# zeyadmohamedabdo/Visual-Question-Answering-VQA-system

Hardware: AMD Instinct MI355X
Metric: image-question pairs/sec (train step) (higher is better)
Workload: dtype bf16; 1 GPU; VQA train step fwd+CE+bwd+allreduce+clip+AdamW, batch 512/GPU, 3x224x224 images, 20 tokens, d=256, 4 text layers, 49 image tokens, 1000 answers, dropout on (BASELINE configs[2]); batch_per_gpu=512, global_batch=512, parallelism=dp1, reducer=off

## Files before the change

include/vqa_hip.h:

```cpp
#ifndef VQA_HIP_H
#define VQA_HIP_H
#include <stdint.h>
#ifdef __cplusplus
extern "C" {
#endif
typedef struct ihipStream_t* hipStream_t;

int vqa_igemm_mtiles(int M, int N, int loader);
int vqa_igemm_variant(int dtype, int loader, int M, int N, int Kw, int B, int H, int W, int C, int Ho, int Wo,
                      int R, int S, int stride, int pad);
int vqa_igemm(int dtype, int loader, const void* a, const void* w, void* out, const float* bias, const void* addend,
              const void* addmask, const void* outmask , float* stats, int M, int N, int Kw, int B, int H, int W, int C, int Ho, int Wo,
              int R, int S, int stride, int pad, int transposed, int relu, float drop_p, unsigned long long drop_seed,
              int stats_mode ,
              hipStream_t stream);
int vqa_linear_dgrad_act(int dtype, const void* dz, const void* wt, void* dx, const void* addend, const void* outact, float drop_p,
                         int M, int Kin, int N, hipStream_t stream);
int vqa_wgrad_plan(int dtype, int loader, int M, int N, int Kw, int B, int H, int W, int C, int R, int S, long long* ws_floats,
                   int* kind, int* tile_n, int* tile_k, int* nsplit);
int vqa_wgrad(int dtype, int loader, const void* dy, const void* x, float* dw, int M, int N, int Kw, int B, int H, int W,
              int C, int Ho, int Wo, int R, int S, int stride, int pad, float* ws, long long ws_floats, hipStream_t stream);
int vqa_pack_rows(int dtype, const float* in, void* out, int N, int K, int Kp, hipStream_t stream);
int vqa_pack_transpose(int dtype, const float* in, void* out, int N, int T, int C, int ldo, int col0, int flip, hipStream_t stream);
int vqa_pack_transpose_batch(int dtype, const float* flat, void* out, const long long* desc, int nd, int total_blocks, hipStream_t stream);
int vqa_fold_bn_batch(int dtype, const float* flat, void* wout, float* bout, const long long* desc, int nd, int total_blocks, float eps, hipStream_t stream);
int vqa_mx_quant(int dtype, const void* in, uint8_t* q, uint8_t* s, int M, int C, hipStream_t stream);
int vqa_fold_bn_mxfp8(const float* flat, uint8_t* wq, uint8_t* ws, float* bout, const long long* desc, int nd, int total_blocks, float eps,
                      hipStream_t stream);
int vqa_conv_mxfp8(const uint8_t* a, const uint8_t* as, const uint8_t* w, const uint8_t* ws, const float* bias, const void* addend,
                   void* out, uint8_t* oq, uint8_t* os, int M, int N, int B, int H, int W, int C, int Ho, int Wo, int R, int S,
                   int stride, int pad, int relu, hipStream_t stream);
int vqa_conv3x3_c64p_blocks(int B, int H, int W);
int vqa_conv3x3_c64p_bnred(const void* x, const void* w, void* out, const void* bn_y, const float* bn_coef, unsigned long long* bn_facc,
                           int B, int H, int W, hipStream_t stream);
int vqa_conv3x3_c64p_epi(const void* x, const void* w, void* out, const void* addend, const void* addmask, const void* outmask,
                         int B, int H, int W, hipStream_t stream);
int vqa_conv3x3_c64p(const void* x, const void* w, void* out, float* stats, int B, int H, int W,
                     int stats_mode , hipStream_t stream);
int vqa_gemm8p(const void* A, const void* B, void* C, int M, int N, int K, hipStream_t stream);
int vqa_gemm4w(const void* A, const void* B, void* C, int M, int N, int K, hipStream_t stream);
int vqa_conv8p_ok(int B, int H, int W, int C, int N);
int vqa_conv8p(const void* x, const void* w, void* out, unsigned long long* stats,
               const void* addend, const void* addmask, const void* outmask ,
               const void* bn_y, const float* bn_coef, unsigned long long* bn_facc ,
               int bn_selfmask ,
               const void* bn_y2, const float* bn_coef2 ,
               int B, int H, int W, int C, int N, int transposed, int stride , hipStream_t stream);
int vqa_conv3x3_c64p_bn(const void* y, const unsigned long long* acc, const float* gamma, const float* beta, float* running_mean,
                        float* running_var, long long* num_batches_tracked, float* coef_out, const void* w, void* out, float* stats,
                        int B, int H, int W, int stats_mode, double count, float momentum, float eps, hipStream_t stream);
int vqa_wgrad3x3_c64_bn_ok(int B, int H, int W);
int vqa_wgrad3x3_c64_bn(const void* y, const float* coef, const void* dy, float* dw , int B, int H, int W,
                        float* ws , long long ws_floats, hipStream_t stream);
int vqa_wgrad3x3_c128_blocks(int B, int H, int W);
int vqa_wgrad3x3_c128(const void* x, const void* dy, float* dw, int B, int H, int W, float* ws, long long ws_floats, hipStream_t stream);
int vqa_wgrad3x3_c64_blocks(int B, int H, int W);
int vqa_wgrad3x3_c64(const void* x, const void* dy, float* dw , int B, int H, int W,
                     float* ws ,
                     long long ws_floats, hipStream_t stream);
long long vqa_wgrad_group_ws(int dtype, int njobs, const int* M, const int* N, const int* Kw);
int vqa_wgrad_group(int dtype, int njobs, const void* const* dy, const void* const* x, float* const* dw, const int* M, const int* N,
                    const int* Kw, float* ws, long long ws_floats, hipStream_t stream);
int vqa_slab_reduce(const float* ws, float* dw, int nslabs, long long n, hipStream_t stream);
int vqa_dgrad_s2(int dtype, const void* dy, const void* dyd, const void* wt, void* out, int B, int H, int W, int C,
                 int Ho, int Wo, int N, int R, int pad, hipStream_t stream);
int vqa_stem_conv_blocks(int B, int H, int W);
int vqa_stem_pack(const float* w_krsc, void* wstem, hipStream_t stream);
int vqa_stem_conv(const float* img, const void* wstem, void* out, float* stats, int B, int H, int W, hipStream_t stream);
int vqa_stem_conv_pool_ok(int B, int H, int W);
int vqa_stem_conv_pool(const float* img, const void* wstem, const float* coef, void* out, int B, int H, int W, hipStream_t stream);
int vqa_stem_wgrad_blocks(int B, int H, int W);
int vqa_stem_wgrad(const float* img, const void* dy, float* dw , int B, int H, int W,
                   float* ws , long long ws_floats, hipStream_t stream);
int vqa_stem_wgrad_fused(const float* img, const void* y, const void* dpool, const uint8_t* idx, const float* coef,
                         const float* bcoef, float* dw, int B, int H, int W, float* ws, long long ws_floats, hipStream_t stream);
int vqa_u8_norm_table(float mean0, float mean1, float mean2, float std0, float std1, float std2, void* table, hipStream_t stream);
int vqa_stem_conv_u8(const uint8_t* img_hwc, const void* wstem, void* out, float* stats, int B, int H, int W, const void* table,
                     hipStream_t stream);
int vqa_stem_conv_pool_u8(const uint8_t* img_hwc, const void* wstem, const float* coef, void* out, int B, int H, int W, const void* table,
                          hipStream_t stream);
int vqa_stem_wgrad_u8(const uint8_t* img_hwc, const void* dy, float* dw, int B, int H, int W, float* ws, long long ws_floats,
                      const void* table, hipStream_t stream);
int vqa_stem_wgrad_fused_u8(const uint8_t* img_hwc, const void* y, const void* dpool, const uint8_t* idx, const float* coef,
                            const float* bcoef, float* dw, int B, int H, int W, float* ws, long long ws_floats, const void* table,
                            hipStream_t stream);
int vqa_stem_dgrad_pack(int dtype, const float* w_krsc, void* wpk, hipStream_t stream);
int vqa_stem_dgrad(int dtype, const void* dy, const void* wpk, float* dimg, int B, int H, int W, hipStream_t stream);
int vqa_stem_dgrad_fused_ok(int B, int H, int W);
int vqa_stem_dgrad_fused(const void* y, const void* dpool, const uint8_t* idx, const float* coef, const float* bcoef, const void* wpk,
                         float* dimg, int B, int H, int W, hipStream_t stream);

int vqa_bn_stats_finalize(const float* part, int tiles, int C, double count, const float* gamma, const float* beta,
                          float* running_mean, float* running_var, long long* num_batches_tracked, float momentum, float eps,
                          double* scratch , float* coef, hipStream_t stream);
int vqa_bn_eval_coef(int C, const float* gamma, const float* beta, const float* running_mean, const float* running_var,
                     float eps, float* coef, hipStream_t stream);
int vqa_bn_apply(int dtype, const void* y, const float* coef, const void* res, const float* rcoef, void* out,
                 long long numel, int C, int relu, hipStream_t stream);
int vqa_bn_apply_pool_chunks(int dtype, int HW, int C);
int vqa_bn_apply_pool(int dtype, const void* y, const float* coef, const void* res, const float* rcoef, void* out, int B, int HW, int C,
                      int relu, float* part, hipStream_t stream);
int vqa_bn_acc_words(int K, int C);
int vqa_bn_apply_acc(int dtype, const void* y, const unsigned long long* acc, const float* gamma, const float* beta, float* running_mean,
                     float* running_var, long long* num_batches_tracked, float* coef_out, const void* res,
                     const unsigned long long* racc, const float* rgamma, const float* rbeta, float* rrunning_mean, float* rrunning_var,
                     long long* rnum_batches_tracked, float* rcoef_out, void* out, int B, int HW, int C, int relu, double count,
                     float momentum, float eps, float* pool_part, hipStream_t stream);
int vqa_bn_bwd_blocks(long long rows);
int vqa_bn_bwd_reduce(int dtype, const void* dout, const void* outact, const void* y, const float* coef, const void* y2,
                      const float* coef2, float* slab , long long rows,
                      int C, int self_mask , int acc_mode, hipStream_t stream);
int vqa_bn_bwd_apply_acc(int dtype, const void* dout, const void* outact, const void* y, const unsigned long long* facc, const float* gamma,
                         const float* coef, float* dgamma, float* dbeta, void* dy, const void* y2, const float* gamma2, const float* coef2,
                         float* dgamma2, float* dbeta2, void* dy2, long long numel, int C, double count, int self_mask, hipStream_t stream);
int vqa_bn_bwd_finalize(const float* slab, int nblk, int C, int which, double count, const float* gamma, const float* coef,
                        int training, float* dgamma, float* dbeta, float* bcoef , hipStream_t stream);
int vqa_bn_bwd_apply(int dtype, const void* dout, const void* outact, const void* y, const float* bcoef, void* dy,
                     const void* y2, const float* bcoef2, void* dy2, long long numel, int C, const float* mask_coef ,
// ... 213 lines not shown
```

visual-question-answering-vqa-system_amd/_lib.py:

```python
from __future__ import annotations

import ctypes as C
import os

import torch

_HERE = os.path.dirname(os.path.abspath(__file__))
LIB_PATH = os.path.join(_HERE, "libvqa_hip.so")

P, I, F, D, LL, ULL = C.c_void_p, C.c_int, C.c_float, C.c_double, C.c_longlong, C.c_ulonglong

SIGNATURES = {
    "vqa_gemm8p": [P, P, P, I, I, I, P],
    "vqa_gemm4w": [P, P, P, I, I, I, P],
    "vqa_conv8p_ok": [I, I, I, I, I],
    "vqa_conv8p": [P, P, P, P, P, P, P, P, P, P, I, P, P, I, I, I, I, I, I, I, P],
    "vqa_igemm_mtiles": [I, I, I],
    "vqa_igemm_variant": [I] * 15,
    "vqa_igemm": [I, I, P, P, P, P, P, P, P, P] + [I] * 15 + [F, ULL, I, P],
    "vqa_linear_dgrad_act": [I, P, P, P, P, P, F, I, I, I, P],
    "vqa_wgrad_plan": [I] * 11 + [P, P, P, P, P],
    "vqa_wgrad": [I, I, P, P, P] + [I] * 13 + [P, LL, P],
    "vqa_pack_rows": [I, P, P, I, I, I, P],
    "vqa_pack_transpose": [I, P, P, I, I, I, I, I, I, P],
    "vqa_pack_transpose_batch": [I, P, P, P, I, I, P],
    "vqa_fold_bn_batch": [I, P, P, P, P, I, I, F, P],
    "vqa_mx_quant": [I, P, P, P, I, I, P],
    "vqa_fold_bn_mxfp8": [P, P, P, P, P, I, I, F, P],
    "vqa_conv_mxfp8": [P] * 9 + [I] * 13 + [P],
    "vqa_conv3x3_c64p_blocks": [I, I, I],
    "vqa_conv3x3_c64p": [P, P, P, P, I, I, I, I, P],
    "vqa_conv3x3_c64p_epi": [P, P, P, P, P, P, I, I, I, P],
    "vqa_conv3x3_c64p_bnred": [P, P, P, P, P, P, I, I, I, P],
    "vqa_conv3x3_c64p_bn": [P, P, P, P, P, P, P, P, P, P, P, I, I, I, I, D, F, F, P],
    "vqa_wgrad3x3_c64_bn_ok": [I, I, I],
    "vqa_wgrad3x3_c64_bn": [P, P, P, P, I, I, I, P, LL, P],
    "vqa_wgrad3x3_c128_blocks": [I, I, I],
    "vqa_wgrad3x3_c128": [P, P, P, I, I, I, P, LL, P],
    "vqa_wgrad3x3_c64_blocks": [I, I, I],
    "vqa_wgrad3x3_c64": [P, P, P, I, I, I, P, LL, P],
    "vqa_wgrad_group_ws": [I, I, P, P, P],
    "vqa_wgrad_group": [I, I, P, P, P, P, P, P, P, LL, P],
    "vqa_slab_reduce": [P, P, I, LL, P],
    "vqa_dgrad_s2": [I, P, P, P, P, I, I, I, I, I, I, I, I, I, P],
    "vqa_stem_conv_blocks": [I, I, I],
    "vqa_stem_pack": [P, P, P],
    "vqa_stem_conv": [P, P, P, P, I, I, I, P],
    "vqa_stem_conv_pool_ok": [I, I, I],
    "vqa_stem_conv_pool": [P, P, P, P, I, I, I, P],
    "vqa_stem_wgrad_blocks": [I, I, I],
    "vqa_stem_wgrad": [P, P, P, I, I, I, P, LL, P],
    "vqa_stem_wgrad_fused": [P, P, P, P, P, P, P, I, I, I, P, LL, P],
    "vqa_u8_norm_table": [F, F, F, F, F, F, P, P],
    "vqa_stem_conv_u8": [P, P, P, P, I, I, I, P, P],
    "vqa_stem_conv_pool_u8": [P, P, P, P, I, I, I, P, P],
    "vqa_stem_wgrad_u8": [P, P, P, I, I, I, P, LL, P, P],
    "vqa_stem_wgrad_fused_u8": [P, P, P, P, P, P, P, I, I, I, P, LL, P, P],
    "vqa_stem_dgrad_pack": [I, P, P, P],
    "vqa_stem_dgrad": [I, P, P, P, I, I, I, P],
    "vqa_stem_dgrad_fused_ok": [I, I, I],
    "vqa_stem_dgrad_fused": [P, P, P, P, P, P, P, I, I, I, P],
    "vqa_bn_stats_finalize": [P, I, I, D, P, P, P, P, P, F, F, P, P, P],
    "vqa_bn_eval_coef": [I, P, P, P, P, F, P, P],
    "vqa_bn_apply": [I, P, P, P, P, P, LL, I, I, P],
    "vqa_bn_apply_pool_chunks": [I, I, I],
    "vqa_bn_apply_pool": [I, P, P, P, P, P, I, I, I, I, P, P],
    "vqa_se_bwd_blocks": [I, I, I, I],
    "vqa_se_bwd_scratch": [I, I, I, I, I],
    "vqa_bn_bwd_blocks": [LL],
    "vqa_bn_bwd_reduce": [I, P, P, P, P, P, P, P, LL, I, I, I, P],
    "vqa_bn_acc_words": [I, I],
    "vqa_bn_apply_acc": [I, P, P, P, P, P, P, P, P, P, P, P, P, P, P, P, P, P, I, I, I, I, D, F, F, P, P],
    "vqa_bn_bwd_apply_acc": [I, P, P, P, P, P, P, P, P, P, P, P, P, P, P, P, LL, I, D, I, P],
    "vqa_bn_bwd_finalize": [P, I, I, I, D, P, P, I, P, P, P, P],
    "vqa_bn_bwd_apply": [I, P, P, P, P, P, P, P, P, LL, I, P, P],
    "vqa_stem_pool_fwd": [I, P, P, P, P, I, I, I, I, P],
    "vqa_stem_bwd_apply": [I, P, P, P, P, P, P, I, I, I, I, P],
    "vqa_se_fwd": [I, P, P, P, P, P, P, P, I, I, I, I, P, I, P],
    "vqa_se_bwd": [I, P, P, P, P, P, P, P, P, P, P, P, I, I, I, I, I, P, P, P, I, P],
    "vqa_spatial_fwd": [I, P, P, P, P, P, P, I, I, I, I, P],
    "vqa_spatial_bwd_scratch": [I, I, I],
    "vqa_spatial_bwd": [I, P, P, P, P, P, P, P, P, P, I, I, I, I, P],
    "vqa_nhwc_to_nchw": [I, P, P, I, I, I, P],
    "vqa_nchw_to_nhwc": [I, P, P, I, I, I, P],
    "vqa_embed_fwd": [I, P, P, P, P, I, I, I, I, F, F, ULL, P],
    "vqa_embed_bwd": [I, P, P, P, I, I, I, F, F, ULL, P],
    "vqa_layernorm_fwd": [I, P, P, P, P, P, I, I, F, F, ULL, P, I, P],
    "vqa_layernorm_bwd_ws": [I, I, I, I],
    "vqa_layernorm_bwd": [I, P, P, P, P, P, P, P, P, I, I, F, ULL, P, I, P, I, P],
    "vqa_layernorm_bwd_folds": [I, I, I, I, P],
    "vqa_attention_fwd": [I, P, P, P, I, I, I, P, P, P, I, I, I, I, I, I, F, ULL, P],
    "vqa_attention_fwd_mfma": [P, P, P, I, I, I, P, P, P, I, I, I, I, I, I, F, ULL, P],
    "vqa_attention_fwd_idx": [I, P, P, P, I, I, I, P, I, P, P, P, I, I, I, I, I, I, P],
    "vqa_attention_fwd_mfma_idx": [P, P, P, I, I, I, P, I, P, P, P, I, I, I, I, I, I, P],
    "vqa_attention_bwd": [I, P, I, P, P, P, I, I, I, P, P, P, P, I, I, I, I, I, I, I, I, F, ULL, P],
    "vqa_accuracy_update": [P, P, P, I, I, P],
    "vqa_softmax_topk": [I, P, LL, P, LL, F, P, P, P, I, I, I, P],
# ... 9 lines not shown
    "vqa_masked_pool_bwd": [I, P, I, I, P, P, P, I, I, I, P],
    "vqa_masked_pool_pair_fwd": [I, P, P, P, P, I, I, I, P],
    "vqa_masked_pool_pair_bwd": [I, P, P, P, P, I, I, I, P],
    "vqa_gate_fwd": [I, P, P, P, I, I, P],
    "vqa_gate_bwd": [I, P, P, P, P, P, I, I, P],
    "vqa_add": [I, P, P, P, LL, P],
    "vqa_grad_tap_add": [I, P, P, I, I, I, I, P],
    "vqa_bias_act_bwd_ws": [I, I, I],
    "vqa_bias_act_bwd": [I, P, P, P, P, I, I, F, ULL, P, I, P],
    "vqa_bias_act_bwd_fold_rows": [I, I, I],
    "vqa_fold_group": [I, P, P, P, P, P, P, P, P],
    "vqa_cross_entropy": [I, P, P, P, P, P, I, I, F, P, P, P],
    "vqa_cross_entropy_opts": [I, P, P, P, P, P, I, I, F, P, P, P, LL, I, F, P, P, P],
    "vqa_answer_scores": [P, P, P, P, I, I, I, I, P, P],
    "vqa_cross_entropy_soft": [I, P, P, P, I, P, P, P, I, I, F, P, P, P, P, P],
    "vqa_challenge_accuracy_update": [P, P, P, I, P, I, I, P],
    "vqa_bce_soft": [I, P, P, P, I, P, P, P, I, I, F, P, P, P, P, P],
    "vqa_convert": [I, I, P, P, LL, P],
    "vqa_sumsq": [P, LL, P, P],
    "vqa_image_normalize": [P, P, P, I, I, I, F, F, F, F, F, F, P],
    "vqa_image_color_jitter": [P, P, P, I, I, I, P, P, F, F, F, F, F, F, P, P],
    "vqa_image_resize_ws": [I, P, P, I, I, I],
    "vqa_image_resize": [P, P, P, P, P, I, I, I, I, I, P, P, P, F, F, F, F, F, F, P, LL, P],
    "vqa_pack_tokens": [P, P, P, P, I, I, I, I, I, I, P],
    "vqa_adamw": [P, P, P, P, LL, F, F, F, F, F, LL, P, F, F, P, P, P, P],
    "vqa_sumsq_ranges": [P, P, I, LL, P, P],
    "vqa_adamw_ranges": [P, P, P, P, P, I, LL, F, F, F, F, F, LL, P, F, F, P, P, P, P, I, P, P],
    "vqa_adamw_ema": [P, P, P, P, LL, F, F, F, F, F, LL, P, F, F, P, P, P, P, F, I, P],
    "vqa_adamw_ranges_ema": [P, P, P, P, P, I, LL, F, F, F, F, F, LL, P, F, F, P, P, P, P, I, P, P, F, I, P],
    "vqa_ema_update": [P, P, LL, F, P],
    "vqa_gather_rows": [P, P, P, I, LL, I, P],
    "vqa_bank_batch": [P, LL, I, P, P, P, P, I, I, P, P],
    "vqa_step_state_set": [P, LL, ULL, F, F, F, F, F, F, F, F, I, P],
    "vqa_adamw_dev": [P, P, P, P, LL, P, P, P, P, P, P],
    "vqa_adamw_ema_dev": [P, P, P, P, LL, P, P, P, P, P, P, P],
    "vqa_adamw_ranges_dev": [P, P, P, P, P, I, LL, P, P, P, P, P, P, I, P, P],
    "vqa_adamw_ranges_ema_dev": [P, P, P, P, P, I, LL, P, P, P, P, P, P, I, P, P, P],
    "vqa_group_hyper_set": [P, I, P, P, P],
    "vqa_adamw_groups": [P, P, P, P, P, I, LL, F, F, F, F, F, LL, P, F, F, P, P, P, P, I, P, P, P, P],
    "vqa_adamw_groups_ema": [P, P, P, P, P, I, LL, F, F, F, F, F, LL, P, F, F, P, P, P, P, I, P, P, F, I, P, P, P],
    "vqa_adamw_groups_dev": [P, P, P, P, P, I, LL, P, P, P, P, P, P, I, P, P, P, P],
    "vqa_adamw_groups_ema_dev": [P, P, P, P, P, I, LL, P, P, P, P, P, P, I, P, P, P, P, P],
    "vqa_sumsq_guard": [P, LL, P, P, P, P, P, P],
    "vqa_sumsq_ranges_guard": [P, P, I, LL, P, P, P, P, P, P],
    "vqa_buffers_save": [P, I, P, P],
    "vqa_buffers_restore": [P, I, P, P, P],
    "vqa_nonfinite_scan": [P, P, I, P, P],
    "vqa_class_seed": [I, P, LL, P, P, P, I, I, P],
    "vqa_gradcam": [I, P, P, P, I, I, I, I, P],
    "vqa_attention_map": [P, P, P, I, I, I, I, I, I, P],
    "vqa_heatmap_render": [P, P, P, P, I, I, I, I, I, F, P],
}
_RET_LL = {"vqa_image_resize_ws", "vqa_wgrad_group_ws", "vqa_spatial_bwd_scratch", "vqa_se_bwd_scratch", "vqa_layernorm_bwd_ws", "vqa_bias_act_bwd_ws"}
_NO_STATUS = _RET_LL | {"vqa_wgrad3x3_c64_blocks", "vqa_bn_acc_words", "vqa_bn_apply_pool_chunks", "vqa_se_bwd_blocks", "vqa_wgrad3x3_c128_blocks", "vqa_layernorm_bwd_folds", "vqa_bias_act_bwd_fold_rows", "vqa_conv3x3_c64p_blocks", "vqa_stem_wgrad_blocks", "vqa_igemm_mtiles", "vqa_igemm_variant", "vqa_bn_bwd_blocks", "vqa_stem_conv_blocks", "vqa_stem_conv_pool_ok", "vqa_stem_dgrad_fused_ok", "vqa_wgrad3x3_c64_bn_ok", "vqa_conv8p_ok"}

_lib = None


def lib() -> C.CDLL:
    global _lib
    if _lib is None:
        if not os.path.exists(LIB_PATH):
            raise RuntimeError(f"{LIB_PATH} is missing: build it with __graft_entry__.build() "
                               "(hipcc --offload-arch=gfx950); there is no CPU fallback")
        L = C.CDLL(LIB_PATH)
        for name, args in SIGNATURES.items():
            fn = getattr(L, name)
            fn.argtypes = args
            fn.restype = LL if name in _RET_LL else I
        _lib = L
    return _lib


def ptr(t):
    return None if t is None else t.data_ptr()


def stream() -> int:
    return torch.cuda.current_stream().cuda_stream


_HOOK = [None]


def call(name: str, *args):
    fn = getattr(lib(), name)
    hook = _HOOK[0]
    done = hook(name, args) if hook is not None else None
    rc = fn(*args, stream())
    if done is not None:
        done()
    if rc != 0:
        raise RuntimeError(f"{name} failed with status {rc}" + (" (argument/shape error)" if rc == 1000 else " (hipError_t)"))


def count(name: str, *args) -> int:
    assert name in _NO_STATUS
    return getattr(lib(), name)(*args)


def dt(t_or_dtype) -> int:
    d = t_or_dtype.dtype if isinstance(t_or_dtype, torch.Tensor) else t_or_dtype
    if d == torch.float32:
        return 0
    if d == torch.bfloat16:
        return 1
    raise TypeError(f"unsupported dtype {d}")
# ... 1 lines not shown
```

visual-question-answering-vqa-system_amd/build.py:

```python
import os
import subprocess
import sys

HERE = os.path.dirname(os.path.abspath(__file__))
CSRC = os.path.join(HERE, "csrc")
SOURCES = ["gemm_conv.hip", "cnn_ops.hip", "token_ops.hip", "stem_conv.hip", "conv_c64.hip", "input_ops.hip", "gemm8p.hip", "mxfp8.hip", "stem_dgrad.hip", "feature_ops.hip", "optim_ops.hip", "loss_ops.hip", "attention.hip", "explain_ops.hip", "batchnorm.hip", "bank_ops.hip"]
LIB = os.path.join(HERE, "libvqa_hip.so")
HIPCC = os.environ.get("HIPCC", "/opt/rocm/bin/hipcc")
FLAGS = ["--offload-arch=gfx950", "-O3", "-std=c++17", "-fPIC", "-Wno-unused-result"]


def _stale():
    if not os.path.exists(LIB):
        return True
    t = os.path.getmtime(LIB)
    import glob
    deps = [os.path.join(CSRC, f) for f in SOURCES] + glob.glob(os.path.join(CSRC, "*.h"))
    return any(os.path.getmtime(d) > t for d in deps)


def build_lib(force=False, verbose=True):
    if not force and not _stale():
        return LIB
    objs = []
    procs = []
    for src in SOURCES:
        obj = os.path.join(CSRC, src.replace(".hip", ".o"))
        objs.append(obj)
        cmd = [HIPCC] + FLAGS + ["-c", os.path.join(CSRC, src), "-o", obj]
        if verbose:
            print(" ".join(cmd), flush=True)
        procs.append((cmd, subprocess.Popen(cmd)))
    for cmd, p in procs:
        if p.wait() != 0:
            raise RuntimeError("hipcc failed: " + " ".join(cmd))
    cmd = [HIPCC, "--offload-arch=gfx950", "-shared", "-fPIC", "-o", LIB] + objs
    if verbose:
        print(" ".join(cmd), flush=True)
    subprocess.check_call(cmd)
    return LIB


if __name__ == "__main__":
    build_lib(force="--force" in sys.argv)
    print(LIB)
```

visual-question-answering-vqa-system_amd/engine.py:

```python
from __future__ import annotations

import math
from typing import Callable, Dict, List, Optional

import torch

from . import kernels as K
from . import layout as LY
from . import stepgraph as SG
from ._lib import call, dt, ptr


def _streams_overlap(a: "torch.cuda.Stream", b: "torch.cuda.Stream", cycles: int = 1_500_000) -> bool:
    ea, eb = torch.cuda.Event(), torch.cuda.Event()
    with torch.cuda.stream(a):
        torch.cuda._sleep(cycles)
        ea.record()
    with torch.cuda.stream(b):
        torch.cuda._sleep(1000)
        eb.record()
    eb.synchronize()
    ok = not ea.query()
    ea.synchronize()
    return ok
# ... 20 lines not shown
def _image_shape(images):
    return images.shape_nchw if K.is_byte_images(images) else tuple(images.shape)


def stem_fcoef(gamma: torch.Tensor, beta: torch.Tensor) -> torch.Tensor:
    fcoef = torch.zeros((4, gamma.numel()), device=gamma.device, dtype=torch.float32)
    fcoef[2] = beta
    fcoef[3] = torch.where(gamma.abs() > 1e-20, 1.0 / gamma, torch.zeros_like(gamma))
    return fcoef


class HipEngine:
    def __init__(self, cfg: dict, entries: List[LY.Entry], flat: torch.Tensor, buffers: Dict[str, torch.Tensor],
                 compute_dtype: torch.dtype):
        self.cfg = cfg
        self.entries = entries
        self.E = {e.name: e for e in entries}
        self.flat = flat
        self.buf = buffers
        self.dtype = compute_dtype
        self.seed_base = 0x5EED
        self.seed_rank = None
        self.step_id = 0
        self._seed_src = None
        self.cnn_train_forwards = 0
        self._running = None
        self.wsrc = flat
        self._wsrc_fresh = False
        self._wt: Dict[str, torch.Tensor] = {}
        self._wt_plan: Dict[str, tuple] = {}
        self._wt_table = None
        self._wt_buf = None
        self._wt_gen = 0
        self._deferred = []
        self._keep = []
        self._wgq = []
        self._foldq = []
        self._foldq2 = []
        self._plan = None
        self._bwd_G = None
        self.fuse_act_dgrad = True
        self.fuse_se_pool = True
        self.fuse_se_bnred = True
        self.fuse_bn_finalize = True
        self.fuse_bn_conv = True
        self.use_conv8p = True
        self.conv8p_n_multiple = 128
        self.conv8p_bwd_n_multiple = 128
        self.pack_off_main = True
        self.hoist_cross = True
        self.use_c64p_epi = True
        self.fuse_bn1_reduce = True
        self.use_conv8p_bwd = True
        self._accbuf = None
        self._accpos = 0
        self._stem_fcoef = None
        self.fold_eval = True
        self._fold = None
        self.infer_precision = "bf16"
        self._foldmx = None
        self.stem_w = None
        self.side, self.side2 = pick_concurrent_streams(flat.device, 2) if flat.is_cuda else (None, None)
        self.two_streams = True
        self.capture = None
        self.capture_io = None
        self.fuse_stem_eval = True
        self.mark = None

    def P(self, name):
        e = self.E[name]
        return self.flat[e.offset: e.offset + e.numel]

    def Wm(self, name):
        return LY.mat_of(self.wsrc, self.E[name])

    def _packT(self, key, pieces, rows, ld):
        t = self._wt.get(key)
        if t is None:
            t = torch.empty((rows, ld), device=self.flat.device, dtype=self.dtype)
            for off, n, tt, c, col0, flip in pieces:
                K.pack_transpose(self.flat[off: off + n * tt * c].view(n, tt, c), self.dtype, out=t, ldo=ld, col0=col0, flip=flip)
            self._wt[key] = t
            self._wt_plan[key] = (tuple(pieces), rows, ld)
            self._wt_table = None
        return t

    def Wt(self, name):
        e = self.E[name]
        n, c = e.shape[0], e.shape[1]
        tt = e.numel // (n * c)
        return self._packT(name, [(e.offset, n, tt, c, 0, False)], c, tt * n)

    def _pack_planned(self):
        if not self._wt_plan:
            return
        if self._wt_table is None or self._wt_table[0].device != self.flat.device:
            rowsd, views, dst, blk = [], [], 0, 0
            for key, (pieces, rows, ld) in self._wt_plan.items():
                for off, n, tt, c, col0, flip in pieces:
                    rowsd.append([off, dst, n, tt, c, ld, col0, int(flip), blk, 0])
                    blk += tt * ((n + 31) // 32) * ((c + 31) // 32)
                views.append((key, dst, rows, ld))
                dst += (rows * ld + 7) // 8 * 8
            self._wt_table = (torch.tensor(rowsd, dtype=torch.int64).to(self.flat.device), views, dst, blk, len(rowsd))
            self._wt_buf = torch.empty(dst, device=self.flat.device, dtype=self.dtype)
            self._wt_gen += 1
# ... 1433 lines not shown
        dy2, dyd = K.bn_bwd(dout, out_act, rec["y2"], rec["c2"], self.P(p + ".bn2.weight"), Cout, training,
                            gs(p + ".bn2.weight"), gs(p + ".bn2.bias"),
                            y2=rec.get("yd"), coef2=rec.get("cd"),
                            gamma2=self.P(p + ".downsample.1.weight") if has_ds else None,
                            dgamma2=gs(p + ".downsample.1.weight") if has_ds else None,
                            dbeta2=gs(p + ".downsample.1.bias") if has_ds else None,
                            slab=pre[0] if (pre and not pre_acc) else None, nb=pre[1] if (pre and not pre_acc) else 0,
                            facc=(pre[0] if pre_acc else (self._acc(K.L.count("vqa_bn_acc_words", 3, Cout)) if bacc else None)), facc_filled=pre_acc)
        g2 = rec["g2"]; B, Ho, Wo = g2[0], g2[1], g2[2]
        if not tw2:
            pass
        elif rec["a1"] is None:
            self._off_path([dy2], lambda: K.wgrad3x3_c64_bn(rec["y1"], rec["c1"], dy2, LY.mat_of(G, self.E[p + ".conv2.weight"]), B, Ho, Wo), defer=last)
        elif self._c64w_ok(B, Ho, Wo, Cout, Cout, 3, 1):
            self._off_path([dy2], lambda: K.wgrad3x3_c64(rec["a1"], dy2, LY.mat_of(G, self.E[p + ".conv2.weight"]), B, Ho, Wo), defer=last)
        elif self._c128w_ok(B, Ho, Wo, Cout, Cout, 1):
            self._off_path([dy2], lambda: K.wgrad3x3_c128(rec["a1"], dy2, LY.mat_of(G, self.E[p + ".conv2.weight"]), B, Ho, Wo))
        else:
            self._off_path([dy2], lambda: K.wgrad(dy2, rec["a1"], LY.mat_of(G, self.E[p + ".conv2.weight"]), M, Cout, 9 * Cout, g2, dtype=T))
        facc1 = None
        if self._c64p_ok(B, Ho, Wo, Cout, Cout, 3, 1) and bacc and self.fuse_bn1_reduce:
            facc1 = self._acc(K.L.count("vqa_bn_acc_words", 3, Cout))
            da1 = K.conv3x3_c64p_bnred(dy2, self._wflip(p + ".conv2.weight"), B, Ho, Wo, rec["y1"], rec["c1"], facc1)
        elif self._c64p_ok(B, Ho, Wo, Cout, Cout, 3, 1):
            da1, _, _ = K.conv3x3_c64p(dy2, self._wflip(p + ".conv2.weight"), B, Ho, Wo)
        elif self.use_conv8p_bwd and self._c8p_ok(B, Ho, Wo, Cout, Cout, 3, 1, 1, bwd=True):
            if bacc and self.fuse_bn1_reduce:
                facc1 = self._acc(K.L.count("vqa_bn_acc_words", 3, Cout))
            da1 = K.conv8p(dy2, self.Wt(p + ".conv2.weight"), B, Ho, Wo, Cout, Cout, transposed=1,
                           bnred=(rec["y1"], rec["c1"], facc1) if facc1 is not None else None)
        else:
            geom_d2 = (B, Ho, Wo, Cout, Ho, Wo, 3, 3, 1, 1)
            da1, _, _ = K.igemm(dy2, self.Wt(p + ".conv2.weight"), M, Cout, 9 * Cout, geom_d2, dtype=T, transposed=1)
        dy1, _ = K.bn_bwd(da1, None, rec["y1"], rec["c1"], self.P(p + ".bn1.weight"), Cout, training,
                          gs(p + ".bn1.weight"), gs(p + ".bn1.bias"), self_mask=True,
                          facc=facc1 if facc1 is not None else (self._acc(K.L.count("vqa_bn_acc_words", 3, Cout)) if bacc else None),
                          facc_filled=facc1 is not None)
        g1 = rec["g1"]; H, W, stride = g1[1], g1[2], g1[8]
        if not tw1:
            pass
        elif self._c64w_ok(B, H, W, Cin, Cout, 3, stride):
            self._off_path([dy1], lambda: K.wgrad3x3_c64(rec["x"], dy1, LY.mat_of(G, self.E[p + ".conv1.weight"]), B, H, W), defer=last)
        elif self._c128w_ok(B, H, W, Cin, Cout, stride):
            self._off_path([dy1], lambda: K.wgrad3x3_c128(rec["x"], dy1, LY.mat_of(G, self.E[p + ".conv1.weight"]), B, H, W))
        else:
            self._off_path([dy1], lambda: K.wgrad(dy1, rec["x"], LY.mat_of(G, self.E[p + ".conv1.weight"]), M, Cout, 9 * Cin, g1, dtype=T))
        Md = B * H * W
        geom_d1 = (B, Ho, Wo, Cout, H, W, 3, 3, stride, 1)
        if has_ds:
            gd = rec["gd"]
            if twd:
                self._off_path([dyd], lambda: K.wgrad(dyd, rec["x"], LY.mat_of(G, self.E[p + ".downsample.0.weight"]), M, Cout, Cin, gd, dtype=T))
            if stride == 2 and H % 2 == 0 and W % 2 == 0:
                wt = self._packT(p + ".dgrad2", [(self.E[p + ".conv1.weight"].offset, Cout, 9, Cin, 0, False),
                                                 (self.E[p + ".downsample.0.weight"].offset, Cout, 1, Cin, 9 * Cout, False)], Cin, 10 * Cout)
                dx = K.dgrad_s2(dy1, dyd, wt, B, Ho, Wo, Cout, H, W, Cin, 3, 1, dtype=T)
            else:
                geom_dd = (B, Ho, Wo, Cout, H, W, 1, 1, stride, 0)
                dxd, _, _ = K.igemm(dyd, self.Wt(p + ".downsample.0.weight"), Md, Cin, Cout, geom_dd, dtype=T, transposed=1)
                dx, _, _ = K.igemm(dy1, self.Wt(p + ".conv1.weight"), Md, Cin, 9 * Cout, geom_d1, dtype=T, transposed=1, addend=dxd)
        elif self.use_c64p_epi and self._c64p_ok(B, H, W, Cout, Cin, 3, stride):
            dx = K.conv3x3_c64p_epi(dy1, self._wflip(p + ".conv1.weight"), B, H, W, addend=dout, addmask=out_act, outmask=outmask)
        elif self.use_conv8p_bwd and stride == 1 and self._c8p_ok(B, H, W, Cout, Cin, 3, stride, 1, bwd=True):
            dx = K.conv8p(dy1, self.Wt(p + ".conv1.weight"), B, H, W, Cout, Cin, transposed=1, addend=dout, addmask=out_act, outmask=outmask)
        else:
            dx, _, _ = K.igemm(dy1, self.Wt(p + ".conv1.weight"), Md, Cin, 9 * Cout, geom_d1, dtype=T, transposed=1,
                               addend=dout, addmask=out_act, outmask=outmask)
        if self.capture is not None:
            self.capture[p] = dict(dout=dout, masked=masked, handed=hand is not None, dy2=dy2, dyd=dyd, da1=da1, dy1=dy1, dx=dx)
        return dx
```

visual-question-answering-vqa-system_amd/kernels.py:

```python
from __future__ import annotations

import os

import torch

from . import _lib as L
from ._lib import call, dt, ptr

LOADER_NHWC, LOADER_STEM = 0, 1

PROFILE = None
PROFILE_VARIANTS = []
PROFILE_STAGED = {}


def prof_begin():
    if PROFILE is None:
        return None
    e0 = torch.cuda.Event(enable_timing=True)
    e0.record()
    return e0


def prof_end(e0, sym, flops, nbytes):
# ... 174 lines not shown


def conv8p_ok(B, H, W, C, N) -> bool:
    return L.count("vqa_conv8p_ok", B, H, W, C, N) > 0


def conv8p(x, w, B, H, W, C, N, *, transposed=0, stride=1, stats_acc=None, out=None, addend=None, addmask=None, outmask=None, bnred=None):
    if out is None:
        out = torch.empty((B * ((H - 1) // stride + 1) * ((W - 1) // stride + 1), N), device=x.device, dtype=torch.bfloat16)
    e0 = prof_begin()
    bn_y, bn_coef, bn_facc, bn_self, bn_y2, bn_coef2 = (tuple(bnred) + (True, None, None))[:6] if bnred is not None else (None, None, None, True, None, None)
    call("vqa_conv8p", ptr(x), ptr(w), ptr(out), ptr(stats_acc), ptr(addend), ptr(addmask), ptr(outmask), ptr(bn_y), ptr(bn_coef), ptr(bn_facc),
         int(bool(bn_self)), ptr(bn_y2), ptr(bn_coef2),
         B, H, W, C, N, int(transposed), int(stride))
    if e0 is not None:
        sym = "conv8p_kernel<2, 4>" if N % 256 == 0 else "conv8p_kernel<4, 2>"
        flops = 2.0 * out.shape[0] * N * 9 * C
        e1 = prof_end(e0, sym, flops,
                      (B * H * W * C + out.shape[0] * N * (1 + sum(t is not None for t in (addend, addmask, outmask, bn_y, bn_y2))) + N * 9 * C) * 2)
        PROFILE_VARIANTS.append((sym, "with epilogue inputs" if (addend is not None or outmask is not None or bnred is not None) else "plain",
                                 flops, e0, e1))
        bmp, bn = (224, 256) if N % 256 == 0 else (448, 128)
        rpt = bmp * 7 // 8 if out.shape[0] % (bmp * 7 // 8) == 0 else bmp
        PROFILE_STAGED[sym] = PROFILE_STAGED.get(sym, 0) + (-(-out.shape[0] // rpt)) * (N // bn) * (9 * C // 64) * (bmp + bn) * 128
    return out


def c64w_blocks(B, H, W) -> int:
    return L.count("vqa_wgrad3x3_c64_blocks", B, H, W)


def wgrad3x3_c64(x, dy, dw, B, H, W):
    e0 = prof_begin()
    wsf = c64w_blocks(B, H, W) * 64 * 576
    ws = torch.empty(wsf, device=x.device, dtype=torch.float32)
    call("vqa_wgrad3x3_c64", ptr(x), ptr(dy), ptr(dw), B, H, W, ptr(ws), wsf)
    if e0 is not None:
        prof_end(e0, "wgrad3x3_c64", 2.0 * B * H * W * 64 * 576, 2 * B * H * W * 64 * 2)


def c128_wgrad_blocks(B, H, W):
    return L.count("vqa_wgrad3x3_c128_blocks", B, H, W)


def wgrad3x3_c128(x, dy, dw, B, H, W):
    e0 = prof_begin()
    wsf = c128_wgrad_blocks(B, H, W) * 128 * 576
    ws = torch.empty(wsf, device=x.device, dtype=torch.float32)
    call("vqa_wgrad3x3_c128", ptr(x), ptr(dy), ptr(dw), B, H, W, ptr(ws), wsf)
    if e0 is not None:
        prof_end(e0, "wgrad3x3_c128p_kernel", 2.0 * B * H * W * 128 * 1152, 2 * B * H * W * 128 * 2)


def dgrad_s2(dy, dyd, wt, B, H, W, C, Ho, Wo, N, R, pad, *, dtype):
    out = torch.empty((B * Ho * Wo, N), device=dy.device, dtype=dtype)
    e0 = prof_begin()
    call("vqa_dgrad_s2", dt(dtype), ptr(dy), ptr(dyd), ptr(wt), ptr(out), B, H, W, C, Ho, Wo, N, R, pad)
    if e0 is not None:
        flops = 2.0 * B * H * W * C * N * (R * R + (1 if dyd is not None else 0))
        prof_end(e0, f"igemm_kernel<{_tname(dtype)}, 128, {64 if N <= 64 else 128}, 2, 4, {_bk(dtype)}, 2, 2, 0>", flops,
                 (B * H * W * C * (2 if dyd is not None else 1) + B * Ho * Wo * N) * 2)
    return out


def is_byte_images(x) -> bool:
    return hasattr(x, "shape_nchw") and hasattr(x, "to_float") and hasattr(x, "mean") and hasattr(x, "std")


_U8_TABLES = {}


def u8_norm_table(device, mean, std):
    key = (str(device), tuple(mean), tuple(std))
    t = _U8_TABLES.get(key)
    if t is None:
        if torch.cuda.is_current_stream_capturing():
            raise RuntimeError("u8_norm_table: the table of a new (mean, std) cannot be built while a HIP graph is being captured")
        t = torch.empty((3, 256), device=device, dtype=torch.bfloat16)
        call("vqa_u8_norm_table", *(float(v) for v in mean), *(float(v) for v in std), ptr(t))
        _U8_TABLES[key] = t
    return t


def _img_of(img):
    if is_byte_images(img):
        return ptr(img.data), ptr(u8_norm_table(img.data.device, img.mean, img.std)), 1, "_u8"
    return ptr(img), None, 4, ""


def _img_device(img):
    return img.data.device if is_byte_images(img) else img.device


def stem_wgrad(img, dy, dw, B, H, W):
    Ho, Wo = (H + 6 - 7) // 2 + 1, (W + 6 - 7) // 2 + 1
    ip, tab, esz, sfx = _img_of(img)
    e0 = prof_begin()
    ws, wsf = stem_wgrad_scratch(_img_device(img), B, H, W)
    call("vqa_stem_wgrad" + sfx, ip, ptr(dy), ptr(dw), B, H, W, ptr(ws), wsf, *(() if tab is None else (tab,)))
    if e0 is not None:
        prof_end(e0, f"stem_wgrad{sfx}_kernel<false>", 2.0 * B * Ho * Wo * 64 * 147, B * 3 * H * W * esz + B * Ho * Wo * 64 * 2)


def stem_wgrad_fused(img, y, dpool, idx, coef, bc, dw, B, H, W):
    Ho, Wo = (H + 6 - 7) // 2 + 1, (W + 6 - 7) // 2 + 1
    ip, tab, esz, sfx = _img_of(img)
    e0 = prof_begin()
    ws, wsf = stem_wgrad_scratch(dpool.device, B, H, W)
    call("vqa_stem_wgrad_fused" + sfx, ip, ptr(y), ptr(dpool), ptr(idx), ptr(coef), ptr(bc), ptr(dw), B, H, W, ptr(ws), wsf,
         *(() if tab is None else (tab,)))
    if e0 is not None:
        prof_end(e0, f"stem_wgrad{sfx}_kernel<true>", 2.0 * B * Ho * Wo * 64 * 147, B * 3 * H * W * esz + B * Ho * Wo * 64 * 2 + dpool.numel() * 3)


# ... 480 lines not shown
```

Baseline: 41550 pairs/s.

## Add quad-decomposed stride-2 dgrad kernel that reuses each dy tile across output phases

Adds a new HIP kernel for the stride-2 3x3 transposed-conv dgrad (plus fused 1x1 shortcut). Each input pixel quad is loaded once, and its contribution to the four output phase classes comes from the matching taps, accumulated in separate MFMA accumulators. The kernel uses LDS double buffering with direct buffer-to-LDS loads and a per-CU rows-per-tile heuristic. The goal is to remove the redundant zero-tap work and repeated dy loads of the generic implicit-GEMM path. The cost is a complex new kernel with high register and LDS use, gated by a shape check that falls back to the old path.

```diff
diff --git a/include/vqa_hip.h b/include/vqa_hip.h
--- a/include/vqa_hip.h
+++ b/include/vqa_hip.h
@@ -64,6 +64,9 @@
 int vqa_slab_reduce(const float* ws, float* dw, int nslabs, long long n, hipStream_t stream);
 int vqa_dgrad_s2(int dtype, const void* dy, const void* dyd, const void* wt, void* out, int B, int H, int W, int C,
                  int Ho, int Wo, int N, int R, int pad, hipStream_t stream);
+int vqa_dgrad_s2q_ok(int B, int H, int W, int C, int N, int has_shortcut);
+int vqa_dgrad_s2q(int dtype, const void* dy, const void* dyd, const void* wt, void* out, int B, int H, int W, int C,
+                  int Ho, int Wo, int N, int R, int pad, hipStream_t stream);
 int vqa_stem_conv_blocks(int B, int H, int W);
 int vqa_stem_pack(const float* w_krsc, void* wstem, hipStream_t stream);
 int vqa_stem_conv(const float* img, const void* wstem, void* out, float* stats, int B, int H, int W, hipStream_t stream);
diff --git a/visual-question-answering-vqa-system_amd/_lib.py b/visual-question-answering-vqa-system_amd/_lib.py
--- a/visual-question-answering-vqa-system_amd/_lib.py
+++ b/visual-question-answering-vqa-system_amd/_lib.py
@@ -43,6 +43,8 @@
     "vqa_wgrad_group": [I, I, P, P, P, P, P, P, P, LL, P],
     "vqa_slab_reduce": [P, P, I, LL, P],
     "vqa_dgrad_s2": [I, P, P, P, P, I, I, I, I, I, I, I, I, I, P],
+    "vqa_dgrad_s2q_ok": [I, I, I, I, I, I],
+    "vqa_dgrad_s2q": [I, P, P, P, P, I, I, I, I, I, I, I, I, I, P],
     "vqa_stem_conv_blocks": [I, I, I],
     "vqa_stem_pack": [P, P, P],
     "vqa_stem_conv": [P, P, P, P, I, I, I, P],
@@ -158,7 +160,7 @@
     "vqa_heatmap_render": [P, P, P, P, I, I, I, I, I, F, P],
 }
 _RET_LL = {"vqa_image_resize_ws", "vqa_wgrad_group_ws", "vqa_spatial_bwd_scratch", "vqa_se_bwd_scratch", "vqa_layernorm_bwd_ws", "vqa_bias_act_bwd_ws"}
-_NO_STATUS = _RET_LL | {"vqa_wgrad3x3_c64_blocks", "vqa_bn_acc_words", "vqa_bn_apply_pool_chunks", "vqa_se_bwd_blocks", "vqa_wgrad3x3_c128_blocks", "vqa_layernorm_bwd_folds", "vqa_bias_act_bwd_fold_rows", "vqa_conv3x3_c64p_blocks", "vqa_stem_wgrad_blocks", "vqa_igemm_mtiles", "vqa_igemm_variant", "vqa_bn_bwd_blocks", "vqa_stem_conv_blocks", "vqa_stem_conv_pool_ok", "vqa_stem_dgrad_fused_ok", "vqa_wgrad3x3_c64_bn_ok", "vqa_conv8p_ok"}
+_NO_STATUS = _RET_LL | {"vqa_wgrad3x3_c64_blocks", "vqa_bn_acc_words", "vqa_bn_apply_pool_chunks", "vqa_se_bwd_blocks", "vqa_wgrad3x3_c128_blocks", "vqa_layernorm_bwd_folds", "vqa_bias_act_bwd_fold_rows", "vqa_conv3x3_c64p_blocks", "vqa_stem_wgrad_blocks", "vqa_igemm_mtiles", "vqa_igemm_variant", "vqa_bn_bwd_blocks", "vqa_stem_conv_blocks", "vqa_stem_conv_pool_ok", "vqa_stem_dgrad_fused_ok", "vqa_wgrad3x3_c64_bn_ok", "vqa_conv8p_ok", "vqa_dgrad_s2q_ok"}
 
 _lib = None
 
diff --git a/visual-question-answering-vqa-system_amd/build.py b/visual-question-answering-vqa-system_amd/build.py
--- a/visual-question-answering-vqa-system_amd/build.py
+++ b/visual-question-answering-vqa-system_amd/build.py
@@ -4,7 +4,7 @@
 
 HERE = os.path.dirname(os.path.abspath(__file__))
 CSRC = os.path.join(HERE, "csrc")
-SOURCES = ["gemm_conv.hip", "cnn_ops.hip", "token_ops.hip", "stem_conv.hip", "conv_c64.hip", "input_ops.hip", "gemm8p.hip", "mxfp8.hip", "stem_dgrad.hip", "feature_ops.hip", "optim_ops.hip", "loss_ops.hip", "attention.hip", "explain_ops.hip", "batchnorm.hip", "bank_ops.hip"]
+SOURCES = ["gemm_conv.hip", "cnn_ops.hip", "token_ops.hip", "stem_conv.hip", "conv_c64.hip", "input_ops.hip", "gemm8p.hip", "mxfp8.hip", "stem_dgrad.hip", "feature_ops.hip", "optim_ops.hip", "loss_ops.hip", "attention.hip", "explain_ops.hip", "batchnorm.hip", "bank_ops.hip", "dgrad_s2.hip"]
 LIB = os.path.join(HERE, "libvqa_hip.so")
 HIPCC = os.environ.get("HIPCC", "/opt/rocm/bin/hipcc")
 FLAGS = ["--offload-arch=gfx950", "-O3", "-std=c++17", "-fPIC", "-Wno-unused-result"]
diff --git a/visual-question-answering-vqa-system_amd/csrc/dgrad_s2.hip b/visual-question-answering-vqa-system_amd/csrc/dgrad_s2.hip
--- /dev/null
+++ b/visual-question-answering-vqa-system_amd/csrc/dgrad_s2.hip
@@ -0,0 +1,234 @@
+#include <type_traits>
+#include "common.h"
+
+namespace {
+constexpr int DQ_BM = 256, DQ_BN = 64, DQ_NW = 8;
+constexpr int DQ_A_BYTES = DQ_BM * 128;
+constexpr int DQ_B_BYTES = 4 * DQ_BN * 128;
+constexpr int DQ_BUF = DQ_A_BYTES + DQ_B_BYTES;
+constexpr int DQ_LDC = 4 * DQ_BN * 2 + 16;
+constexpr int DQ_LDS = 2 * DQ_BUF > DQ_BM * DQ_LDC ? 2 * DQ_BUF : DQ_BM * DQ_LDC;
+constexpr int DQ_OOB = (int)0x80000000;
+static_assert(DQ_LDS <= 160 * 1024 && DQ_BM == DQ_NW * 32, "LDS budget / wave split");
+
+__host__ __device__ constexpr int dq_tap(int src, int cls) {
+  return src == 0 ? (cls == 3 ? 0 : -1)
+       : src == 1 ? (cls == 2 ? 1 : cls == 3 ? 2 : -1)
+       : src == 2 ? (cls == 1 ? 3 : cls == 3 ? 6 : -1)
+       : src == 3 ? (cls == 0 ? 4 : cls == 1 ? 5 : cls == 2 ? 7 : 8)
+       : (cls == 0 ? 9 : -1);
+}
+
+__device__ __forceinline__ int dq_div(int m, unsigned long long mul) { return (int)(((unsigned long long)(unsigned)m * mul) >> 40); }
+}
+
+struct DQParams {
+  const bf16_t* dy; const bf16_t* dyd; const bf16_t* wt; bf16_t* out;
+  int H, W, C, N, Kw, nquads, tiles_n, has_sc;
+  int rpt;
+  unsigned a_bytes, w_bytes;
+  unsigned long long mul_hw, mul_w;
+};
+
+__global__ __launch_bounds__(DQ_NW * 64, 2) void dgrad_s2q_kernel(DQParams p) {
+  extern __shared__ __attribute__((aligned(16))) char smem[];
+  const int tid = threadIdx.x, lane = tid & 63, li = lane & 15, g = lane >> 4;
+  const int w = __builtin_amdgcn_readfirstlane(tid >> 6);
+  int tile;
+  {
+    const int nwg = (int)gridDim.x, orig = (int)blockIdx.x, xcd = orig & 7, q = nwg >> 3, r = nwg & 7;
+    tile = (xcd < r ? xcd * (q + 1) : r * (q + 1) + (xcd - r) * q) + (orig >> 3);
+  }
+  const int tm = tile / p.tiles_n, tn = tile - tm * p.tiles_n;
+  const int m0 = tm * p.rpt, n0 = tn * DQ_BN;
+  const __amdgpu_buffer_rsrc_t rsA = __builtin_amdgcn_make_buffer_rsrc(const_cast<bf16_t*>(p.dy), 0, (int)p.a_bytes, 0x00020000);
+  const __amdgpu_buffer_rsrc_t rsA2 = __builtin_amdgcn_make_buffer_rsrc(const_cast<bf16_t*>(p.has_sc ? p.dyd : p.dy), 0, (int)p.a_bytes, 0x00020000);
+  const __amdgpu_buffer_rsrc_t rsW = __builtin_amdgcn_make_buffer_rsrc(const_cast<bf16_t*>(p.wt), 0, (int)p.w_bytes, 0x00020000);
+
+  const int dr = lane >> 3, dc = lane & 7, slot = (dc ^ dr) << 4;
+  const int csz = p.C * 2;
+  int pixoff[4], aoff[4];
+  unsigned edge = 0;
+#pragma unroll
+  for (int h = 0; h < 4; ++h) {
+    const int lr = w * 32 + h * 8 + dr, q = m0 + lr;
+    pixoff[h] = DQ_OOB;
+    if (lr < p.rpt && q < p.nquads) {
+      const int b = dq_div(q, p.mul_hw), rem = q - b * p.H * p.W, i = dq_div(rem, p.mul_w), j = rem - i * p.W;
+      pixoff[h] = ((b * p.H + i) * p.W + j) * csz + slot;
+      edge |= (i + 1 < p.H ? 1u : 0u) << (2 * h) | (j + 1 < p.W ? 2u : 0u) << (2 * h);
+    }
+  }
+  const int boff = (n0 + w * 8 + dr) * p.Kw * 2 + slot;
+  auto set_src = [&](auto src_c) __attribute__((always_inline)) {
+    constexpr int SRC = decltype(src_c)::value;
+    constexpr int dh = (SRC == 0 || SRC == 1) ? 1 : 0, dw = (SRC == 0 || SRC == 2) ? 1 : 0;
+    constexpr unsigned need = (dh ? 1u : 0u) | (dw ? 2u : 0u);
+    const int d = (dh * p.W + dw) * csz;
+#pragma unroll
+    for (int h = 0; h < 4; ++h)
+      aoff[h] = (pixoff[h] >= 0 && ((edge >> (2 * h)) & need) == need) ? pixoff[h] + d : DQ_OOB;
+  };
+  auto load = [&](auto src_c, int cc, int buf) __attribute__((always_inline)) {
+    constexpr int SRC = decltype(src_c)::value;
+#if defined(__HIP_DEVICE_COMPILE__)
+    typedef __attribute__((address_space(3))) void* lds_ptr;
+    char* ab = smem + buf * DQ_BUF + w * 4096;
+#pragma unroll
+    for (int h = 0; h < 4; ++h)
+      if (w * 32 + h * 8 < p.rpt)
+        __builtin_amdgcn_raw_ptr_buffer_load_lds(SRC == 4 ? rsA2 : rsA, (lds_ptr)(ab + h * 1024), 16, aoff[h], cc * 128, 0, 0);
+    char* bb = smem + buf * DQ_BUF + DQ_A_BYTES + w * 1024;
+#pragma unroll
+    for (int c = 0; c < 4; ++c)
+      if (dq_tap(SRC, c) >= 0)
+        __builtin_amdgcn_raw_ptr_buffer_load_lds(rsW, (lds_ptr)(bb + c * (DQ_BN * 128)), 16, boff, (dq_tap(SRC, c) * p.C + cc * 64) * 2, 0, 0);
+#else
+    (void)cc; (void)buf;
+#endif
+  };
+
+  f32x4 acc[4][2][4];
+#pragma unroll
+  for (int c = 0; c < 4; ++c)
+#pragma unroll
+    for (int i = 0; i < 2; ++i)
+#pragma unroll
+      for (int j = 0; j < 4; ++j) acc[c][i][j] = f32x4{0.f, 0.f, 0.f, 0.f};
+
+  const int rswz = lane & 7;
+  auto compute = [&](auto src_c, int buf) __attribute__((always_inline)) {
+    constexpr int SRC = decltype(src_c)::value;
+    const char* Ab = smem + buf * DQ_BUF + (w * 32 + li) * 128;
+    const char* Bb = smem + buf * DQ_BUF + DQ_A_BYTES + li * 128;
+#pragma unroll
+    for (int kk = 0; kk < 2; ++kk) {
+      const int so = ((kk * 4 + g) ^ rswz) * 16;
+      bf16x8 af[2];
+#pragma unroll
+      for (int i = 0; i < 2; ++i) af[i] = *reinterpret_cast<const bf16x8*>(Ab + i * 2048 + so);
+#pragma unroll
+      for (int c = 0; c < 4; ++c) {
+        if (dq_tap(SRC, c) < 0) continue;
+        bf16x8 bfv[4];
+#pragma unroll
+        for (int j = 0; j < 4; ++j) bfv[j] = *reinterpret_cast<const bf16x8*>(Bb + c * (DQ_BN * 128) + j * 2048 + so);
+#pragma unroll
+        for (int i = 0; i < 2; ++i)
+#pragma unroll
+          for (int j = 0; j < 4; ++j)
+            acc[c][i][j] = __builtin_amdgcn_mfma_f32_16x16x32_bf16(bfv[j], af[i], acc[c][i][j], 0, 0, 0);
+      }
+    }
+  };
+  auto wait_barrier = [&]() __attribute__((always_inline)) { asm volatile("s_waitcnt vmcnt(0) lgkmcnt(0)\n\ts_barrier" ::: "memory"); };
+
+  const int cpb = p.C / 64;
+  int buf = 0;
+  set_src(std::integral_constant<int, 0>{});
+  load(std::integral_constant<int, 0>{}, 0, 0);
+  wait_barrier();
+  auto run_src = [&](auto src_c, bool more) __attribute__((always_inline)) {
+    constexpr int SRC = decltype(src_c)::value;
+    for (int cc = 0; cc < cpb; ++cc) {
+      if (cc + 1 < cpb) load(src_c, cc + 1, buf ^ 1);
+      else if (SRC < 4 && more) {
+        set_src(std::integral_constant<int, (SRC < 4 ? SRC + 1 : 4)>{});
+        load(std::integral_constant<int, (SRC < 4 ? SRC + 1 : 4)>{}, 0, buf ^ 1);
+      }
+      if (w * 32 < p.rpt) compute(src_c, buf);
+      wait_barrier();
+      buf ^= 1;
+    }
+  };
+  run_src(std::integral_constant<int, 0>{}, true);
+  run_src(std::integral_constant<int, 1>{}, true);
+  run_src(std::integral_constant<int, 2>{}, true);
+  run_src(std::integral_constant<int, 3>{}, p.has_sc != 0);
+  if (p.has_sc) run_src(std::integral_constant<int, 4>{}, false);
+
+  typedef __attribute__((ext_vector_type(2))) float f32x2_t;
+  typedef __attribute__((ext_vector_type(2))) __bf16 bf16x2_t;
+  typedef __attribute__((ext_vector_type(2))) uint32_t u32x2_t;
+#pragma unroll
+  for (int c = 0; c < 4; ++c)
+#pragma unroll
+    for (int i = 0; i < 2; ++i)
+#pragma unroll
+      for (int j = 0; j < 4; ++j) {
+        const bf16x2_t lo = __builtin_convertvector((f32x2_t){acc[c][i][j][0], acc[c][i][j][1]}, bf16x2_t);
+        const bf16x2_t hi = __builtin_convertvector((f32x2_t){acc[c][i][j][2], acc[c][i][j][3]}, bf16x2_t);
+        *reinterpret_cast<u32x2_t*>(smem + (w * 32 + i * 16 + li) * DQ_LDC + c * 128 + j * 32 + g * 8) =
+            u32x2_t{__builtin_bit_cast(uint32_t, lo), __builtin_bit_cast(uint32_t, hi)};
+      }
+  __syncthreads();
+  const int cls = dr & 3, ph = cls >> 1, pw = cls & 1;
+  const int Ho = 2 * p.H, Wo = 2 * p.W;
+#pragma unroll 4
+  for (int t = 0; t < 16; ++t) {
+    const int rl = w * 32 + 2 * t + (dr >> 2), q = m0 + rl;
+    if (rl < p.rpt && q < p.nquads) {
+      const int b = dq_div(q, p.mul_hw), rem = q - b * p.H * p.W, i = dq_div(rem, p.mul_w), j = rem - i * p.W;
+      const size_t m = (size_t)(b * Ho + 2 * i + ph) * Wo + 2 * j + pw;
+      const u32x4 v = *reinterpret_cast<const u32x4*>(smem + rl * DQ_LDC + cls * 128 + dc * 16);
+      *reinterpret_cast<u32x4*>(p.out + m * p.N + n0 + dc * 8) = v;
+    }
+  }
+}
+
+static int dq_cus() {
+  static int ncu = 0;
+  if (ncu == 0) {
+    int dev = 0, n = 0;
+    ncu = (hipGetDevice(&dev) == hipSuccess && hipDeviceGetAttribute(&n, hipDeviceAttributeMultiprocessorCount, dev) == hipSuccess && n > 0) ? n : 256;
+  }
+  return ncu;
+}
+static int dq_rows_per_tile(int nquads, int tiles_n, int cpb) {
+  const int ncu = dq_cus();
+  int best = DQ_BM; long long best_cost = -1;
+  for (int rpt = DQ_BM; rpt >= DQ_BM / 2; --rpt) {
+    const long long tiles = (long long)((nquads + rpt - 1) / rpt) * tiles_n, rounds = (tiles + ncu - 1) / ncu;
+    const long long cost = rounds * (2ll * cpb * (5 * ((rpt + 7) / 8) + 80) + 3ll * rpt);
+    if (best_cost < 0 || cost < best_cost) { best = rpt; best_cost = cost; }
+  }
+  return best;
+}
+
+extern "C" {
+
+static int dq_can(int B, int H, int W, int C, int N) {
+  if (B <= 0 || H <= 0 || W <= 0 || C <= 0 || N <= 0 || C % 64 || N % DQ_BN) return 0;
+  const unsigned long long nq = (unsigned long long)B * H * W;
+  if (nq * 4ull * N >= (1ull << 31)) return 0;
+  if (nq * C * 2ull >= 0x7fffffffull || (unsigned long long)N * 10ull * C * 2ull >= 0x7fffffffull) return 0;
+  if ((nq + DQ_BM) * (unsigned long long)(H * W) >= (1ull << 40)) return 0;
+  return 1;
+}
+
+int vqa_dgrad_s2q_ok(int B, int H, int W, int C, int N, int has_shortcut) {
+  (void)has_shortcut;
+  if (!dq_can(B, H, W, C, N)) return 0;
+  if (N == 128 && (long long)((B * H * W + DQ_BM - 1) / DQ_BM) * (N / DQ_BN) > dq_cus()) return 0;
+  return 1;
+}
+
+int vqa_dgrad_s2q(int dtype, const void* dy, const void* dyd, const void* wt, void* out, int B, int H, int W, int C,
+                  int Ho, int Wo, int N, int R, int pad, hipStream_t st) {
+  if (!dy || !wt || !out || dtype != 1 || R != 3 || pad != 1 || Ho != 2 * H || Wo != 2 * W) return VQA_EARG;
+  if (!dq_can(B, H, W, C, N)) return VQA_EARG;
+  DQParams p;
+  p.dy = (const bf16_t*)dy; p.dyd = (const bf16_t*)dyd; p.wt = (const bf16_t*)wt; p.out = (bf16_t*)out;
+  p.H = H; p.W = W; p.C = C; p.N = N; p.Kw = 9 * C + (dyd ? C : 0); p.nquads = B * H * W; p.tiles_n = N / DQ_BN; p.has_sc = dyd ? 1 : 0;
+  p.a_bytes = (unsigned)((size_t)p.nquads * C * 2); p.w_bytes = (unsigned)((size_t)N * p.Kw * 2);
+  const unsigned long long one = 1ull << 40, hw = (unsigned long long)H * W;
+  p.mul_hw = (one + hw - 1) / hw; p.mul_w = (one + (unsigned long long)W - 1) / (unsigned long long)W;
+  p.rpt = dq_rows_per_tile(p.nquads, p.tiles_n, C / 64);
+  const int tiles = ((p.nquads + p.rpt - 1) / p.rpt) * p.tiles_n;
+  (void)vqa_ensure_lds(reinterpret_cast<const void*>(&dgrad_s2q_kernel), DQ_LDS);
+  hipLaunchKernelGGL(dgrad_s2q_kernel, dim3(tiles), dim3(DQ_NW * 64), DQ_LDS, st, p);
+  VQA_LAUNCH_CHECK();
+  return VQA_OK;
+}
+
+}
diff --git a/visual-question-answering-vqa-system_amd/engine.py b/visual-question-answering-vqa-system_amd/engine.py
--- a/visual-question-answering-vqa-system_amd/engine.py
+++ b/visual-question-answering-vqa-system_amd/engine.py
@@ -96,6 +96,7 @@
         self.use_c64p_epi = True
         self.fuse_bn1_reduce = True
         self.use_conv8p_bwd = True
+        self.use_dgrad_s2_quad = True
         self._accbuf = None
         self._accpos = 0
         self._stem_fcoef = None
@@ -1635,9 +1636,9 @@
             if twd:
                 self._off_path([dyd], lambda: K.wgrad(dyd, rec["x"], LY.mat_of(G, self.E[p + ".downsample.0.weight"]), M, Cout, Cin, gd, dtype=T))
             if stride == 2 and H % 2 == 0 and W % 2 == 0:
-                wt = self._packT(p + ".dgrad2", [(self.E[p + ".conv1.weight"].offset, Cout, 9, Cin, 0, False),
+                wt =self._packT(p + ".dgrad2", [(self.E[p + ".conv1.weight"].offset, Cout, 9, Cin, 0, False),
                                                  (self.E[p + ".downsample.0.weight"].offset, Cout, 1, Cin, 9 * Cout, False)], Cin, 10 * Cout)
-                dx = K.dgrad_s2(dy1, dyd, wt, B, Ho, Wo, Cout, H, W, Cin, 3, 1, dtype=T)
+                dx = K.dgrad_s2(dy1, dyd, wt, B, Ho, Wo, Cout, H, W, Cin, 3, 1, dtype=T, quad=None if self.use_dgrad_s2_quad else False)
             else:
                 geom_dd = (B, Ho, Wo, Cout, H, W, 1, 1, stride, 0)
                 dxd, _, _ = K.igemm(dyd, self.Wt(p + ".downsample.0.weight"), Md, Cin, Cout, geom_dd, dtype=T, transposed=1)
diff --git a/visual-question-answering-vqa-system_amd/kernels.py b/visual-question-answering-vqa-system_amd/kernels.py
--- a/visual-question-answering-vqa-system_amd/kernels.py
+++ b/visual-question-answering-vqa-system_amd/kernels.py
@@ -250,14 +250,24 @@
         prof_end(e0, "wgrad3x3_c128p_kernel", 2.0 * B * H * W * 128 * 1152, 2 * B * H * W * 128 * 2)
 
 
-def dgrad_s2(dy, dyd, wt, B, H, W, C, Ho, Wo, N, R, pad, *, dtype):
+def dgrad_s2q_ok(B, H, W, C, N, has_shortcut, *, dtype, R=3, pad=1, Ho=None, Wo=None) -> bool:
+    if dtype != torch.bfloat16 or R != 3 or pad != 1 or (Ho is not None and Ho != 2 * H) or (Wo is not None and Wo != 2 * W):
+        return False
+    if "vqa_dgrad_s2q_ok" not in L.SIGNATURES:
+        return False
+    return L.count("vqa_dgrad_s2q_ok", B, H, W, C, N, int(bool(has_shortcut))) > 0
+
+
+def dgrad_s2(dy, dyd, wt, B, H, W, C, Ho, Wo, N, R, pad, *, dtype, quad=None):
+    if quad is None:
+        quad = dgrad_s2q_ok(B, H, W, C, N, dyd is not None, dtype=dtype, R=R, pad=pad, Ho=Ho, Wo=Wo)
     out = torch.empty((B * Ho * Wo, N), device=dy.device, dtype=dtype)
     e0 = prof_begin()
-    call("vqa_dgrad_s2", dt(dtype), ptr(dy), ptr(dyd), ptr(wt), ptr(out), B, H, W, C, Ho, Wo, N, R, pad)
+    call("vqa_dgrad_s2q" if quad else "vqa_dgrad_s2", dt(dtype), ptr(dy), ptr(dyd), ptr(wt), ptr(out), B, H, W, C, Ho, Wo, N, R, pad)
     if e0 is not None:
         flops = 2.0 * B * H * W * C * N * (R * R + (1 if dyd is not None else 0))
-        prof_end(e0, f"igemm_kernel<{_tname(dtype)}, 128, {64 if N <= 64 else 128}, 2, 4, {_bk(dtype)}, 2, 2, 0>", flops,
-                 (B * H * W * C * (2 if dyd is not None else 1) + B * Ho * Wo * N) * 2)
+        sym = "dgrad_s2q_kernel" if quad else f"igemm_kernel<{_tname(dtype)}, 128, {64 if N <= 64 else 128}, 2, 4, {_bk(dtype)}, 2, 2, 0>"
+        prof_end(e0, sym, flops, (B * H * W * C * (2 if dyd is not None else 1) + B * Ho * Wo * N) * 2)
     return out
 
 
```

Measured after the change: 41540 pairs/s. No clear change (-0.0%).
